# theovincent/iS-DQN

Hardware: AMD Instinct MI355X
Metric: gradient-steps/sec (batch=256, K=9, 84x84x4) (higher is better)
Workload: dtype bf16x3 (split-bf16 MFMA operands hi+lo, fp32 accumulate)

## Files before the change

is-dqn_amd/csrc/net_kernels.hip:

```cpp
#include <stdarg.h>
#include <stdlib.h>

#include <algorithm>
#include <type_traits>
#include <vector>
#include <atomic>

#include "conv_img.h"
#include "conv_u8_pair.h"
#include "conv_s8_pair.h"
#include "head_loss.h"
#include "munchausen.h"
#include "hl_gauss.h"
#include "quantile.h"
#include "categorical.h"
#include "net_plan.h"
#include "net_problems.h"

namespace isdqn {

__device__ inline double pow_int(double b, int t) {
    double r = 1.0, x = b;
    for (unsigned u = (unsigned)t; u != 0; u >>= 1) {
        if (u & 1u) r *= x;
// ... 315 lines not shown
    double* __restrict__ priorities = args.priorities;
    extern __shared__ float s_d[];
    __shared__ int s_action[TD_ROWS];
    const int tid = threadIdx.x, lane = tid & 63, wave = tid >> 6;
    const int b0 = blockIdx.x * TD_ROWS;
    const int b = b0 + lane;
    const bool on = b < B;
    float* s_td = s_d + TD_ROWS * K;
    const float inv_b = 1.f / (float)B;
    if (dout != nullptr) {
        const int rows = min(TD_ROWS, B - b0);
        for (int i = tid; i < rows * nha_p; i += 256) dout[(int64_t)b0 * nha_p + i] = 0.f;
    }
    int a = 0;
    float r = 0.f, nt = 0.f, w = 1.f;
    if (on) {
        a = action[b];
        r = reward[b];
        nt = 1.f - (float)terminal[b];
        if (loss_weights != nullptr) w = loss_weights[b];
    }
    if (wave == 0) s_action[lane] = on ? a : -1;
    for (int k = wave; k < K; k += 4) {
        float d = 0.f, td = 0.f;
        if (on) {
            float qv = q[(int64_t)b * nha_p + (oh + k) * A + a];
            const float* nq = vq + (int64_t)b * nha_p + (th + k) * A;
            float mx = nq[0];
            if (sq != nullptr) {
                const float* sel = sq + (int64_t)b * sq_pitch + (sh + k) * A;
                ISDQN_BOUNDS_CHECK(sel, 4 * A, 30);
                ISDQN_BOUNDS_CHECK(nq, 4 * A, 30);
                mx = nq[argmax_first(sel, A)];
            } else {
                for (int j = 1; j < A; ++j) mx = fmaxf(mx, nq[j]);
            }
            float tg = r + nt * gamma_n * mx;
            if (mq != nullptr) {
                const float* sv = mq + (int64_t)b * mq_pitch + (mh + k) * A;
                ISDQN_BOUNDS_CHECK(sv, 4 * A, 31);
                ISDQN_BOUNDS_CHECK(nq, 4 * A, 31);
                tg = munchausen_target(r, nt, gamma_n, sv[a], soft_value(sv, A, mu.tau), soft_value(nq, A, mu.tau), mu);
            }
            d = qv - tg;
            td = td_loss(d, huber_delta);
            if (q_values) q_values[(int64_t)b * K + k] = qv;
            if (targets) targets[(int64_t)b * K + k] = tg;
        }
        s_d[lane * K + k] = td_dloss(d, huber_delta) * inv_b * w;
        s_td[lane * K + k] = td;
        float sum = td * w;
        for (int off = 32; off > 0; off >>= 1) sum += __shfl_xor(sum, off);
        if (lane == 0) loss_part[(int64_t)blockIdx.x * K + k] = sum;
    }
    __syncthreads();
    if (dout != nullptr) {
        for (int i = tid; i < TD_ROWS * K; i += 256) {
            int bl = i / K, k = i - bl * K;
            if (b0 + bl < B) dout[(int64_t)(b0 + bl) * nha_p + (oh + k) * A + s_action[bl]] = s_d[i];
        }
        for (int c = tid; c < nha_p; c += 256) {
            float sum = 0.f;
            int head = c / A, aa = c - head * A;
            if (head >= oh && head < oh + K)
                for (int bl = 0; bl < TD_ROWS; ++bl) sum += (s_action[bl] == aa) ? s_d[bl * K + head - oh] : 0.f;
            dbh_part[(int64_t)blockIdx.x * nha_p + c] = sum;
        }
    }
    if (priorities != nullptr && tid < TD_ROWS && b0 + tid < B) {
        float sum = 0.f;
        for (int k = 0; k < K; ++k) sum += s_td[tid * K + k];
        priorities[b0 + tid] = sqrt((double)(sum / (float)K) + 1e-10);
    }
}

struct HeadChainParams {
    const float* slabs;
    int n_slabs;
    int64_t slab_stride, row_pitch;
    const float* hbias;
    float* act;
    float* z;
    const float* W;
    const float* bias;
    const float* gamma;
    const float* beta;
    int B, S, F, Fp, O, Op, K, A, oh;
    const int* action;
    const float* reward;
    const uint8_t* terminal;
    const float* loss_weights;
    float gamma_n, huber_delta;
    int double_q;
    Munchausen mu;
    float* dout;
    float* dz;
    float* part;
    float* q_values;
    float* targets;
    double* priorities;
    float* loss_part;
    float* dbh_part;
    int* adam_count;
    float b1, b2;
    float* adam_consts;
    long long* stamps;
};

constexpr int HC_MAX_COLS = 4;
constexpr int HC_THREADS = 512, HC_WAVES = HC_THREADS / 64;
constexpr int HC_KU = 16 / HC_WAVES;

__host__ __device__ inline int head_chain_pitch(int Fp) { return (Fp + 31) / 32 * 32 + 8; }
static inline int head_chain_lds_bytes(int Fp, int Op, int K, int passes, int S) {
    const int PA = head_chain_pitch(Fp);
    return (passes >= 2 ? 2 : 1) * 16 * PA * 2 + (HC_WAVES * 16 * Op + 16 * Op + S * Op + Op + 4 + 2 * S * Fp) * 4 + S * K * 12 +
           HC_WAVES * 2 * S * 2 * 4 + 64;
}

template <int PASSES, int COLS, int SMAX>
__global__ __launch_bounds__(HC_THREADS) void head_chain_kernel(const HeadChainParams p) {
    ISDQN_EMPTY_KERNEL_RETURN
    extern __shared__ __attribute__((aligned(16))) char hc_smem[];
    const int PA = head_chain_pitch(p.Fp);
    constexpr int A_PLANES = PASSES >= 2 ? 2 : 1;
    __bf16* a_hi = reinterpret_cast<__bf16*>(hc_smem);
    __bf16* a_lo = a_hi + 16 * PA;
    float* qpart = reinterpret_cast<float*>(a_hi + A_PLANES * 16 * PA);
    float* s_q = qpart + HC_WAVES * 16 * p.Op;
    float* s_dq = s_q + 16 * p.Op;
    float* s_d = s_dq + SMAX * p.Op;
    float* s_td = s_d + SMAX * p.K;
    float* s_wtd = s_td + SMAX * p.K;
    float* s_red = s_wtd + SMAX * p.K;
    float* s_bias = s_red + HC_WAVES * 2 * SMAX * 2;
    float* s_pre = reinterpret_cast<float*>((reinterpret_cast<uintptr_t>(s_bias + p.Op) + 15) & ~(uintptr_t)15);

    const int tid = threadIdx.x, lane = tid & 63, wave = tid >> 6;
#if defined(ISDQN_DEV)
#define HC_STAMP(i)                                                                                     \
    if (p.stamps != nullptr && threadIdx.x == 0) {                                                     \
        p.stamps[(int64_t)blockIdx.x * 8 + (i)] = (long long)__builtin_amdgcn_s_memtime();              \
        if ((i) == 0) p.stamps[(int64_t)blockIdx.x * 8 + 7] = (long long)__builtin_amdgcn_s_memrealtime(); \
    }
#else
#define HC_STAMP(i)
#endif
    HC_STAMP(0);
    const int S = p.S, b0 = (int)blockIdx.x * S;
    const int Fp = p.Fp, Op = p.Op, K = p.K, A = p.A;

    if (blockIdx.x == 0 && tid == 0) {
        int t = *p.adam_count + 1;
        *p.adam_count = t;
        p.adam_consts[0] = (float)(1.0 - pow_int((double)p.b1, t));
        p.adam_consts[1] = (float)(1.0 - pow_int((double)p.b2, t));
    }

    int act[SMAX];
#pragma unroll
    for (int s = 0; s < SMAX; ++s) {
        ISDQN_BOUNDS_CHECK((s < S && b0 + s < p.B) ? (const void*)(p.action + b0 + s) : zero_chunk(), 4, 20);
        act[s] = *(const ISDQN_GLOBAL int*)((s < S && b0 + s < p.B) ? (const void*)(p.action + b0 + s) : zero_chunk());
    }
    float td_r, td_w;
    uint8_t td_term;
    {
        const int s = tid / K;
        const bool ok = tid < S * K && b0 + s < p.B;
        const bool okw = ok && p.loss_weights != nullptr;
        ISDQN_BOUNDS_CHECK(okw ? (const void*)(p.loss_weights + b0 + s) : zero_chunk(), 4, 29);
        td_w = *(const ISDQN_GLOBAL float*)(okw ? (const void*)(p.loss_weights + b0 + s) : zero_chunk());
        ISDQN_BOUNDS_CHECK(ok ? (const void*)(p.reward + b0 + s) : zero_chunk(), 4, 21);
        ISDQN_BOUNDS_CHECK(ok ? (const void*)(p.terminal + b0 + s) : zero_chunk(), 1, 22);
        td_r = *(const ISDQN_GLOBAL float*)(ok ? (const void*)(p.reward + b0 + s) : zero_chunk());
        td_term = *(const ISDQN_GLOBAL uint8_t*)(ok ? (const void*)(p.terminal + b0 + s) : zero_chunk());
    }
    ISDQN_BOUNDS_CHECK(tid < p.O ? (const void*)(p.bias + tid) : zero_chunk(), 4, 23);
    const float bias_v = *(const ISDQN_GLOBAL float*)(tid < p.O ? (const void*)(p.bias + tid) : zero_chunk());
    float ga[COLS], be[COLS];
#pragma unroll
    for (int j = 0; j < COLS; ++j) {
        const int c = tid + j * HC_THREADS;
        const bool ok = p.gamma != nullptr && c < p.F;
        ISDQN_BOUNDS_CHECK(ok ? (const void*)(p.gamma + c) : zero_chunk(), 4, 24);
        ISDQN_BOUNDS_CHECK(ok ? (const void*)(p.beta + c) : zero_chunk(), 4, 24);
        ga[j] = *(const ISDQN_GLOBAL float*)(ok ? (const void*)(p.gamma + c) : zero_chunk());
        be[j] = *(const ISDQN_GLOBAL float*)(ok ? (const void*)(p.beta + c) : zero_chunk());
    }

    constexpr int R2 = 2 * SMAX;
    constexpr int TPR = HC_THREADS / R2;
    constexpr int SB = 32;
    static_assert(TPR % 64 == 0, "a wave must not straddle two rows");
    float m1 = 0.f, m2 = 0.f;
    {
        const int r = tid / TPR, q = tid - r * TPR;
        const int smp = r < S ? r : r - S;
        const bool row_ok = r < 2 * S && b0 + smp < p.B;
        const int64_t grow = r < S ? (int64_t)(b0 + smp) : (int64_t)p.B + b0 + smp;
        for (int c0 = q * 4; c0 < Fp; c0 += TPR * 4) {
            float hb4[4];
#pragma unroll
            for (int e = 0; e < 4; ++e) {
                ISDQN_BOUNDS_CHECK(c0 + e < p.F ? (const void*)(p.hbias + c0 + e) : zero_chunk(), 4, 25);
                hb4[e] = *(const ISDQN_GLOBAL float*)(c0 + e < p.F ? (const void*)(p.hbias + c0 + e) : zero_chunk());
            }
            const ISDQN_GLOBAL f32x4* base = (const ISDQN_GLOBAL f32x4*)(row_ok ? (const void*)(p.slabs + grow * p.row_pitch + c0) : zero_chunk());
            const int64_t strd = row_ok ? p.slab_stride / 4 : 0;
            f32x4 sum = f32x4{0.f, 0.f, 0.f, 0.f};
            for (int s0 = 0; s0 < p.n_slabs; s0 += SB) {
                f32x4 t[SB];
#pragma unroll
                for (int u = 0; u < SB; ++u) {
                    ISDQN_BOUNDS_CHECK((const void*)(base + min(s0 + u, p.n_slabs - 1) * strd), 16, 26);
                    t[u] = base[min(s0 + u, p.n_slabs - 1) * strd];
                }
#pragma unroll
                for (int u = 0; u < SB; ++u)
                    if (s0 + u < p.n_slabs) sum += t[u];
            }
            float v[4];
#pragma unroll
            for (int e = 0; e < 4; ++e) {
                v[e] = c0 + e < p.F ? sum[e] + hb4[e] : 0.f;
                m1 += v[e];
                m2 += v[e] * v[e];
            }
            *reinterpret_cast<float4*>(s_pre + r * Fp + c0) = make_float4(v[0], v[1], v[2], v[3]);
        }
    }

    HC_STAMP(6);
    const int nkt = (PA - 8) / 32, NT = (Op + 15) / 16;
    const int nks = (nkt + 15) / 16, n_items = ((NT + 1) / 2) * nks;
    const int kg8 = (lane >> 4) * 8;
    const int arow = (lane & 15) * PA + kg8;
    auto issue_w = [&](float (&v)[2][HC_KU][8], int item) {
        const int pair = item / nks, ksb = wave + 16 * (item - pair * nks);
#pragma unroll
        for (int t = 0; t < 2; ++t)
#pragma unroll
            for (int u = 0; u < HC_KU; ++u) {
                const int o = (pair * 2 + t) * 16 + (lane & 15), ks = ksb + HC_WAVES * u;
                const bool ok = item < n_items && o < p.O && ks < nkt && ks * 32 + kg8 < Fp;
                load8_aligned(ok ? p.W + (int64_t)o * Fp + ks * 32 + kg8 : zero_chunk(), v[t][u]);
            }
    };
    float wv0[2][HC_KU][8], wv1[2][HC_KU][8];
    issue_w(wv0, 0);

    float zv[SMAX][COLS];
    {
        for (int off = 32; off > 0; off >>= 1) {
            m1 += __shfl_xor(m1, off);
            m2 += __shfl_xor(m2, off);
        }
        if (lane == 0) {
            s_red[wave * 2] = m1;
            s_red[wave * 2 + 1] = m2;
        }
        __syncthreads();
        constexpr int WPR = TPR / 64;
#pragma unroll
        for (int r = 0; r < R2; ++r) {
            float a1 = s_red[r * WPR * 2], a2 = s_red[r * WPR * 2 + 1];
#pragma unroll
            for (int w = 1; w < WPR; ++w) {
                a1 += s_red[(r * WPR + w) * 2];
                a2 += s_red[(r * WPR + w) * 2 + 1];
            }
            const float mean = a1 / (float)p.F;
            const float rstd = rsqrtf(fmaxf(a2 / (float)p.F - mean * mean, 0.f) + 1e-6f);
            const int smp = r < S ? r : r - S;
            const bool row_ok = r < 2 * S && b0 + smp < p.B;
            const int64_t grow = r < S ? (int64_t)(b0 + smp) : (int64_t)p.B + b0 + smp;
#pragma unroll
            for (int j = 0; j < COLS; ++j) {
                const int c = tid + j * HC_THREADS;
                const float v = c < Fp ? s_pre[r * Fp + c] : 0.f;
                float y = v;
                if (p.gamma != nullptr && c < p.F) y = (v - mean) * (rstd * ga[j]) + be[j];
                y = fmaxf(y, 0.f);
                if (c >= p.F) y = 0.f;
                if (row_ok && c < Fp) {
                    s8_store_elem(p.act + grow * Fp, c, y);
                    if (r < S) p.z[grow * Fp + c] = v;
                }
                if (r < 2 * S && c < PA - 8) {
                    const float ys = row_ok ? y : 0.f;
                    const __bf16 h = (__bf16)ys;
                    a_hi[r * PA + c] = h;
                    if constexpr (PASSES >= 2) a_lo[r * PA + c] = (__bf16)(ys - (float)h);
                }
                if (r < SMAX) zv[r < SMAX ? r : 0][j] = (row_ok && r < S && c < p.F) ? v : 0.f;
            }
        }
    }
    for (int i = tid; i < SMAX * Op; i += HC_THREADS) s_dq[i] = 0.f;
    if (tid < Op) s_bias[tid] = bias_v;
    for (int o = tid + HC_THREADS; o < Op; o += HC_THREADS) s_bias[o] = o < p.O ? p.bias[o] : 0.f;
    __syncthreads();
    HC_STAMP(1);

    {
        f32x4 acc[2];
        auto run_item = [&](float (&v)[2][HC_KU][8], int item) {
            const int pair = item / nks, ksi = item - pair * nks, ksb = wave + 16 * ksi;
            if (ksi == 0) {
                acc[0] = acc[1] = f32x4{0.f, 0.f, 0.f, 0.f};
            }
#pragma unroll
            for (int u = 0; u < HC_KU; ++u) {
                const int ks = min(ksb + HC_WAVES * u, nkt - 1);
                const bf16x8 ah = *reinterpret_cast<const bf16x8*>(a_hi + arow + ks * 32);
                bf16x8 al;
                if constexpr (PASSES >= 2) al = *reinterpret_cast<const bf16x8*>(a_lo + arow + ks * 32);
#pragma unroll
                for (int t = 0; t < 2; ++t) {
                    bf16x8 bh, bl;
                    if constexpr (PASSES >= 2) {
                        split8(v[t][u], bh, bl);
                        if constexpr (PASSES >= 3)
                            mfma_acc(acc[t], ah, bl);
                        mfma_acc(acc[t], al, bh);
                    } else {
                        round8(v[t][u], bh);
                    }
                    mfma_acc(acc[t], ah, bh);
                }
            }
            const bool last = ksi + 1 == nks;
            if (last) {
#pragma unroll
                for (int t = 0; t < 2; ++t) {
                    const int o = (pair * 2 + t) * 16 + (lane & 15);
                    if (o < Op) {
#pragma unroll
                        for (int r = 0; r < 4; ++r) qpart[(wave * 16 + (lane >> 4) * 4 + r) * Op + o] = acc[t][r];
                    }
                }
            }
        };
        for (int item = 0; item < n_items; item += 2) {
            issue_w(wv1, item + 1);
            run_item(wv0, item);
            issue_w(wv0, item + 2);
            if (item + 1 < n_items) run_item(wv1, item + 1);
        }
    }

    auto issue_rows = [&](float (&w)[SMAX][4][COLS], int k0) {
#pragma unroll
        for (int s = 0; s < SMAX; ++s)
#pragma unroll
            for (int u = 0; u < 4; ++u) {
                const bool on = s < S && k0 + u < K;
                const float* wr = p.W + (int64_t)(on ? (p.oh + k0 + u) * A + act[s] : 0) * Fp;
#pragma unroll
                for (int j = 0; j < COLS; ++j) {
                    const int c = tid + j * HC_THREADS;
                    ISDQN_BOUNDS_CHECK(wr + (c < p.F ? c : 0), 4, 27);
                    w[s][u][j] = *(const ISDQN_GLOBAL float*)(wr + (c < p.F ? c : 0));
                }
            }
    };
    HC_STAMP(2);
    float wr0[SMAX][4][COLS], wr1[SMAX][4][COLS];
    issue_rows(wr0, 0);
    __syncthreads();
    for (int i = tid; i < 2 * S * Op; i += HC_THREADS) {
        const int o = i % Op;
        float v = qpart[i];
#pragma unroll
        for (int w = 1; w < HC_WAVES; ++w) v += qpart[w * 16 * Op + i];
        s_q[i] = o < p.O ? v + s_bias[o] : 0.f;
    }
    __syncthreads();

    const float inv_b = 1.f / (float)p.B;
    if (tid < S * K) {
        const int s = tid / K, k = tid - s * K;
        const int b = b0 + s;
        float d = 0.f, td = 0.f;
        int a = 0;
        if (b < p.B) {
            a = act[0];
#pragma unroll
            for (int i = 1; i < SMAX; ++i) a = s == i ? act[i] : a;
            const float qv = s_q[s * Op + (p.oh + k) * A + a];
            const float* nq = s_q + (S + s) * Op + k * A;
            float mx = nq[0];
            if (p.double_q) {
                mx = nq[argmax_first(nq + p.oh * A, A)];
            } else {
                for (int j = 1; j < A; ++j) mx = fmaxf(mx, nq[j]);
            }
            float tg = td_r + (1.f - (float)td_term) * p.gamma_n * mx;
            if (p.mu.tau > 0.f) {
                const float* sv = s_q + s * Op + k * A;
                tg = munchausen_target(td_r, 1.f - (float)td_term, p.gamma_n, sv[a], soft_value(sv, A, p.mu.tau), soft_value(nq, A, p.mu.tau), p.mu);
            }
            d = qv - tg;
            td = td_loss(d, p.huber_delta);
            if (p.q_values) p.q_values[(int64_t)b * K + k] = qv;
            if (p.targets) p.targets[(int64_t)b * K + k] = tg;
        }
        const float w = p.loss_weights != nullptr ? td_w : 1.f;
        const float dd = td_dloss(d, p.huber_delta) * inv_b * w;
        s_d[tid] = dd;
        s_td[tid] = td;
        s_wtd[tid] = td * w;
        s_dq[s * Op + (p.oh + k) * A + a] = dd;
    }
    __syncthreads();
    for (int i = tid; i < S * Op; i += HC_THREADS) {
        const int s = i / Op;
        if (b0 + s < p.B) p.dout[(int64_t)b0 * Op + i] = s_dq[i];
    }
    for (int c = tid; c < Op; c += HC_THREADS) {
        float sum = 0.f;
        for (int s = 0; s < S; ++s) sum += s_dq[s * Op + c];
        p.dbh_part[(int64_t)blockIdx.x * Op + c] = sum;
    }
    if (tid < K) {
        float sum = 0.f;
        for (int s = 0; s < S; ++s) sum += s_wtd[s * K + tid];
        p.loss_part[(int64_t)blockIdx.x * K + tid] = sum;
    }
    if (p.priorities != nullptr && tid < S && b0 + tid < p.B) {
        float sum = 0.f;
        for (int k = 0; k < K; ++k) sum += s_td[tid * K + k];
        p.priorities[b0 + tid] = sqrt((double)(sum / (float)K) + 1e-10);
    }

    HC_STAMP(3);
    float da[SMAX][COLS];
#pragma unroll
    for (int s = 0; s < SMAX; ++s)
#pragma unroll
        for (int j = 0; j < COLS; ++j) da[s][j] = 0.f;
    auto axpy_rows = [&](const float (&w)[SMAX][4][COLS], int k0) {
#pragma unroll
        for (int s = 0; s < SMAX; ++s)
#pragma unroll
            for (int u = 0; u < 4; ++u) {
                const bool on = s < S && k0 + u < K;
                const float dd = on ? s_d[s * K + k0 + u] : 0.f;
#pragma unroll
                for (int j = 0; j < COLS; ++j) da[s][j] += dd * w[s][u][j];
            }
    };
    for (int k0 = 0; k0 < K; k0 += 8) {
        issue_rows(wr1, k0 + 4);
        axpy_rows(wr0, k0);
        issue_rows(wr0, k0 + 8);
        if (k0 + 4 < K) axpy_rows(wr1, k0 + 4);
    }
    HC_STAMP(4);
    float dg[COLS], db[COLS], dbias[COLS];
#pragma unroll
    for (int j = 0; j < COLS; ++j) dg[j] = db[j] = dbias[j] = 0.f;
    if (p.gamma != nullptr) {
        const float inv_c = 1.f / (float)p.F;
        float r1[SMAX], r2[SMAX];
        auto block_sum2 = [&]() {
#pragma unroll
            for (int s = 0; s < SMAX; ++s)
                for (int off = 32; off > 0; off >>= 1) {
                    r1[s] += __shfl_xor(r1[s], off);
                    r2[s] += __shfl_xor(r2[s], off);
                }
            __syncthreads();
            if (lane == 0) {
#pragma unroll
                for (int s = 0; s < SMAX; ++s) {
                    s_red[(wave * SMAX + s) * 2] = r1[s];
                    s_red[(wave * SMAX + s) * 2 + 1] = r2[s];
                }
            }
            __syncthreads();
#pragma unroll
            for (int s = 0; s < SMAX; ++s) {
                r1[s] = s_red[s * 2];
                r2[s] = s_red[s * 2 + 1];
#pragma unroll
                for (int w = 1; w < HC_WAVES; ++w) {
                    r1[s] += s_red[(w * SMAX + s) * 2];
                    r2[s] += s_red[(w * SMAX + s) * 2 + 1];
                }
            }
        };
#pragma unroll
        for (int s = 0; s < SMAX; ++s) {
            r1[s] = r2[s] = 0.f;
#pragma unroll
            for (int j = 0; j < COLS; ++j) {
                r1[s] += zv[s][j];
                r2[s] += zv[s][j] * zv[s][j];
            }
        }
        block_sum2();
        float mean[SMAX], rstd[SMAX];
#pragma unroll
        for (int s = 0; s < SMAX; ++s) {
            mean[s] = r1[s] * inv_c;
            rstd[s] = rsqrtf(fmaxf(r2[s] * inv_c - mean[s] * mean[s], 0.f) + 1e-6f);
            r1[s] = r2[s] = 0.f;
#pragma unroll
            for (int j = 0; j < COLS; ++j) {
                const int c = tid + j * HC_THREADS;
                const bool ok = c < p.F && s < S && b0 + s < p.B;
                const float xh = (zv[s][j] - mean[s]) * rstd[s];
                const float y = xh * ga[j] + be[j];
                const float dy = (ok && y > 0.f) ? da[s][j] : 0.f;
                dg[j] += dy * xh;
                db[j] += dy;
                const float g2 = dy * ga[j];
                da[s][j] = g2;
                zv[s][j] = ok ? xh : 0.f;
                r1[s] += g2;
                r2[s] += g2 * zv[s][j];
            }
        }
        block_sum2();
#pragma unroll
        for (int s = 0; s < SMAX; ++s) {
            const float m1 = r1[s] * inv_c, m2 = r2[s] * inv_c;
            if (s < S && b0 + s < p.B) {
#pragma unroll
                for (int j = 0; j < COLS; ++j) {
                    const int c = tid + j * HC_THREADS;
                    if (c < Fp) {
                        const float o = c < p.F ? rstd[s] * (da[s][j] - m1 - zv[s][j] * m2) : 0.f;
                        dbias[j] += o;
                        s8_store_elem(p.dz + (int64_t)(b0 + s) * Fp, c, o);
                    }
                }
            }
        }
    } else {
#pragma unroll
        for (int s = 0; s < SMAX; ++s) {
            if (s < S && b0 + s < p.B) {
#pragma unroll
                for (int j = 0; j < COLS; ++j) {
                    const int c = tid + j * HC_THREADS;
                    if (c < Fp) {
                        const float o = (c < p.F && zv[s][j] > 0.f) ? da[s][j] : 0.f;
                        dbias[j] += o;
                        s8_store_elem(p.dz + (int64_t)(b0 + s) * Fp, c, o);
                    }
                }
            }
        }
    }
#pragma unroll
    for (int j = 0; j < COLS; ++j) {
        const int c = tid + j * HC_THREADS;
        if (c < Fp) {
            float* pp = p.part + (int64_t)blockIdx.x * 3 * Fp;
            pp[c] = dg[j];
            pp[Fp + c] = db[j];
            pp[2 * Fp + c] = dbias[j];
        }
    }
    HC_STAMP(5);
#undef HC_STAMP
}

__global__ __launch_bounds__(256) void loss_finalize_kernel(const float* __restrict__ loss_part,
                                                            const float* __restrict__ dbh_part, int n_blk, int B, int K,
                                                            int nha_p, float* __restrict__ losses,
                                                            float* __restrict__ loss_accum, float* __restrict__ dbh,
                                                            int* adam_count, float b1, float b2,
                                                            float* __restrict__ adam_consts) {
    ISDQN_EMPTY_KERNEL_RETURN
    const int tid = threadIdx.x, sub = tid & 15, grp = tid >> 4;
    const int nkb = (K + 15) / 16;
    const bool is_loss = (int)blockIdx.x < nkb;
    const int col = (is_loss ? (int)blockIdx.x : (int)blockIdx.x - nkb) * 16 + grp;
    const int ncol = is_loss ? K : nha_p;
    const float* src = is_loss ? loss_part : dbh_part;
    if (!is_loss && dbh == nullptr) return;
    float s = 0.f;
    if (col < ncol)
        for (int i0 = sub; i0 < n_blk; i0 += 8 * 16) {
            float v[8];
#pragma unroll
            for (int u = 0; u < 8; ++u) {
                const int i = i0 + u * 16;
                v[u] = i < n_blk ? src[(int64_t)i * ncol + col] : 0.f;
            }
#pragma unroll
            for (int u = 0; u < 8; ++u) s += v[u];
        }
    for (int off = 8; off > 0; off >>= 1) s += __shfl_xor(s, off);
    if (col < ncol && sub == 0) {
        if (is_loss) {
            s /= (float)B;
            losses[col] = s;
            if (loss_accum != nullptr) loss_accum[col] += s;
        } else {
            dbh[col] = s;
        }
    }
    if (blockIdx.x != 0) return;
    if (adam_count != nullptr && tid == 0) {
        int t = *adam_count + 1;
        *adam_count = t;
        adam_consts[0] = (float)(1.0 - pow_int((double)b1, t));
        adam_consts[1] = (float)(1.0 - pow_int((double)b2, t));
    }
}

struct AdamEntry {
    int64_t p_off, size, slab_stride;
    const float* g;
    int n_slabs, block_start;
};
constexpr int ADAM_MAX_ENTRIES = 4 * MAX_LAYERS;
struct AdamTable {
    AdamEntry e[ADAM_MAX_ENTRIES];
    int n, total_blocks;
};
__global__ __launch_bounds__(256) void adam_kernel(const AdamTable tab, float* __restrict__ p, float* __restrict__ m,
                                                   float* __restrict__ v, const float* __restrict__ consts, float lr,
                                                   float b1, float b2, float eps, float* __restrict__ grad_out,
                                                   float* __restrict__ mirror, int update) {
    ISDQN_EMPTY_KERNEL_RETURN
    __shared__ float4 s_g[16][16];
    int e = 0;
    while (e + 1 < tab.n && (int)blockIdx.x >= tab.e[e + 1].block_start) ++e;
    const AdamEntry en = tab.e[e];
    const float c1 = consts[0], c2 = consts[1];
    const int pos = threadIdx.x & 15, sl = threadIdx.x >> 4;
    const int64_t i = ((int64_t)(blockIdx.x - en.block_start) * 16 + pos) * 4;
    const bool on = i < en.size;
    float4 g = float4{0.f, 0.f, 0.f, 0.f};
    const int64_t o = en.p_off + i;
    float4 pm = g, pv = g, pp = g;
    if (on && sl == 0) {
        pm = *reinterpret_cast<const float4*>(m + o);
        pv = *reinterpret_cast<const float4*>(v + o);
        pp = *reinterpret_cast<const float4*>(p + o);
    }
    if (on) {
        int s = sl;
#if !defined(ISDQN_ADAM_4_IN_FLIGHT)
        for (; s + 7 * 16 < en.n_slabs; s += 8 * 16) {
// ... 955 lines not shown
};

static void head_chain_plan(LearnCtx& c, bool plan_heads) {
    const Plan& P = c.P;
    const Layer& hid = c.hid();
    static const bool hc_disabled = ISDQN_DEV_ENV("ISDQN_NO_HEAD_CHAIN");
    if (!(c.learn && c.update && plan_heads && !hc_disabled && c.target_params == nullptr && P.head_nb == 0 && P.n_layers >= 2 && hid.kind == 1 &&
          !hid.is_head && hid.has_relu && hid.out_p <= HC_THREADS * HC_MAX_COLS && hid.out_p % 8 == 0))
        return;
    const int S = c.B >= 1024 ? 4 : c.B >= 512 ? 2 : 1;
    const int n_wg = ceil_div(c.B, S);
    if (n_wg <= hid.part_rows && S * c.K <= HC_THREADS && head_chain_lds_bytes(hid.out_p, P.nha_p, c.K, c.x3 ? 3 : 1, S) <= 150 * 1024) {
        c.hc_S = S;
        c.hc_wg = n_wg;
    }
}

static int learn_forward(const LearnCtx& c) {
    const Plan& P = c.P;
    const isdqn_batch* batch = c.batch;
    float* ws = c.ws;
    const int B = c.B;
    int rc;
    if (c.target_params != nullptr && c.munchausen) {
        const int stack = c.cfg->arch != ISDQN_ARCH_FC ? c.cfg->obs_c : 0;
        rc = refresh_mirror(P, c.target_params, ws, c.st);
        if (rc) return rc;
        rc = net_forward(P, c.x3, c.target_params, c.in, P.N2, 0, ws, ws + P.out_t_off, c.st);
        if (rc) return rc;
        if (P.head_nb > 0) {
            rc = head_expect_rows(P, ws + P.logits_t_off, P.N2, ws + P.qt_off, c.st);
            if (rc) return rc;
        }
        rc = refresh_mirror(P, c.params, ws, c.st);
        if (rc) return rc;
        NetInput on{batch->frames, batch->frame_stride, batch->frame_ids, 0, batch->state, nullptr, 0, 2 * stack, 0};
        return net_forward(P, c.x3, c.params, on, B, B, ws, ws + P.out_off, c.st);
    }
    if (c.target_params != nullptr && c.double_q) {
        const int stack = c.cfg->arch != ISDQN_ARCH_FC ? c.cfg->obs_c : 0;
        NetInput nx{batch->frames, batch->frame_stride, batch->frame_ids, 0, batch->next_state, nullptr, 0, 2 * stack, stack};
        rc = refresh_mirror(P, c.target_params, ws, c.st);
        if (rc) return rc;
        rc = net_forward(P, c.x3, c.target_params, nx, B, 0, ws, ws + P.out_t_off, c.st);
        if (rc) return rc;
        if (P.head_nb > 0) {
            rc = head_expect_rows(P, ws + P.logits_t_off, B, ws + P.qt_off, c.st);
            if (rc) return rc;
        }
        rc = refresh_mirror(P, c.params, ws, c.st);
        if (rc) return rc;
        return net_forward(P, c.x3, c.params, c.in, P.N2, B, ws, ws + P.out_off, c.st);
    }
    if (c.target_params != nullptr) {
        const int stack = c.cfg->arch != ISDQN_ARCH_FC ? c.cfg->obs_c : 0;
        NetInput nx{batch->frames, batch->frame_stride, batch->frame_ids, 0, batch->next_state, nullptr, 0, 2 * stack, stack};
        rc = refresh_mirror(P, c.target_params, ws, c.st);
        if (rc) return rc;
        rc = net_forward(P, c.x3, c.target_params, nx, B, 0, ws, ws + P.out_off + (int64_t)B * P.nlog_p, c.st);
        if (rc) return rc;
        rc = refresh_mirror(P, c.params, ws, c.st);
        if (rc) return rc;
        NetInput on{batch->frames, batch->frame_stride, batch->frame_ids, 0, batch->state, nullptr, 0, 2 * stack, 0};
        return net_forward(P, c.x3, c.params, on, B, B, ws, ws + P.out_off, c.st);
    }
    if (!(batch->flags & ISDQN_BATCH_MIRROR_CURRENT)) {
        rc = refresh_mirror(P, c.params, ws, c.st);
        if (rc) return rc;
    }
    return net_forward(P, c.x3, c.params, c.in, P.N2, B, ws, ws + P.out_off, c.st, c.hc_S ? P.n_layers - 1 : -1, c.hc_S ? P.n_layers - 2 : -1);
}

static int launch_head_chain(const LearnCtx& c) {
    const Plan& P = c.P;
    const Layer &hid = c.hid(), &head = c.head();
    float* ws = c.ws;
    HeadChainParams hp;
    hp.act = ws + hid.act_off; hp.z = ws + hid.z_off;
    hp.slabs = ws + P.slab_off;
    hp.n_slabs = effective_splits(hid.in_unpadded_ld ? hid.in_f : hid.K, hid.fwd_splits);
    hp.slab_stride = hid.out_p;
    hp.row_pitch = (int64_t)hp.n_slabs * hid.out_p;
    hp.hbias = c.params + hid.b_off;
    hp.W = c.params + head.w_off; hp.bias = c.params + head.b_off;
    hp.gamma = hid.has_ln ? c.params + hid.g_off : nullptr;
    hp.beta = hid.has_ln ? c.params + hid.be_off : nullptr;
    hp.B = c.B; hp.S = c.hc_S; hp.F = hid.out_f; hp.Fp = hid.out_p; hp.O = P.nha; hp.Op = P.nha_p; hp.K = c.K; hp.oh = P.oh;
    hp.A = P.n_actions;
    hp.action = c.batch->action; hp.reward = c.batch->reward; hp.terminal = c.batch->terminal;
    hp.loss_weights = c.batch->loss_weights;
    hp.gamma_n = c.cfg->gamma_n; hp.huber_delta = c.cfg->huber_delta;
    hp.double_q = c.double_q ? 1 : 0;
    hp.mu = Munchausen{c.cfg->munchausen_tau, c.cfg->munchausen_alpha, c.cfg->munchausen_clip};
    hp.dout = ws + P.dout_off; hp.dz = ws + hid.dz_off; hp.part = ws + hid.part_off;
    hp.q_values = c.qv; hp.targets = c.tg; hp.priorities = c.priorities;
    hp.loss_part = ws + P.lpart_off; hp.dbh_part = hp.loss_part + (int64_t)c.hc_wg * c.K;
    hp.adam_count = c.adam_count; hp.b1 = c.cfg->adam_b1; hp.b2 = c.cfg->adam_b2; hp.adam_consts = ws + P.adam_tab_off;
    hp.stamps = stamps_for("head_chain");
    const int lds = head_chain_lds_bytes(hid.out_p, P.nha_p, c.K, c.x3 ? 3 : 1, c.hc_S);
    const int cols = ceil_div(hid.out_p, HC_THREADS) <= 1 ? 1 : ceil_div(hid.out_p, HC_THREADS) <= 2 ? 2 : 4;
    auto launch_hc = [&](auto kern, int slot) -> int {
        static LdsConfigured configured[18];
        if (int rc2 = ensure_dynamic_lds(kern, lds, configured[slot])) return rc2;
        ISDQN_REPORT_OCCUPANCY(kern, HC_THREADS, lds, c.hc_wg);
        hipLaunchKernelGGL(kern, dim3(c.hc_wg), dim3(HC_THREADS), lds, c.st, hp);
        ISDQN_HIP_CHECK(hipGetLastError());
        return ISDQN_OK;
    };
    auto by_cols = [&](auto passes_c, auto s_c, int base) -> int {
        constexpr int PS = decltype(passes_c)::value, SS = decltype(s_c)::value;
        return cols == 1 ? launch_hc(&head_chain_kernel<PS, 1, SS>, base) : cols == 2 ? launch_hc(&head_chain_kernel<PS, 2, SS>, base + 1)
                                                                        : launch_hc(&head_chain_kernel<PS, 4, SS>, base + 2);
    };
    auto by_s = [&](auto passes_c, int base) -> int {
        return c.hc_S == 1 ? by_cols(passes_c, std::integral_constant<int, 1>{}, base)
             : c.hc_S == 2 ? by_cols(passes_c, std::integral_constant<int, 2>{}, base + 3)
                           : by_cols(passes_c, std::integral_constant<int, 4>{}, base + 6);
    };
    return c.x3 ? by_s(std::integral_constant<int, 3>{}, 0) : by_s(std::integral_constant<int, 1>{}, 9);
}

static int head_chain_sums(const LearnCtx& c, hipStream_t s) {
    return loss_finalize(c.P, c.cfg, c.ws, c.hc_wg, c.K, c.P.nha_p, c.losses, c.loss_accum, true, nullptr, s);
}
static int head_chain_tail(const LearnCtx& c, hipStream_t s) {
    if (int rc = head_chain_sums(c, s)) return rc;
    const Layer& head = c.head();
    return dense_wgrad(head, c.x3, c.in, c.ws + c.hid().act_off, c.ws + c.P.dout_off, c.P.nlog_p, c.ws + head.gw_off, c.B, s);
}

static int learn_loss(const LearnCtx& c) {
    const bool tnet = (c.double_q || c.munchausen) && c.target_params != nullptr;
    if (!c.hc_S)
        return loss_and_finalize(c.P, c.cfg, c.ws, c.batch, c.K, c.on0, c.tg0, c.learn, (c.learn && c.update) ? c.adam_count : nullptr, c.qv, c.tg,
                                 c.priorities, c.losses, c.loss_accum, c.st, c.double_q,
                                 tnet ? c.ws + c.P.out_t_off + (c.munchausen ? (int64_t)c.B * c.P.nlog_p : 0) : nullptr,
                                 (tnet && c.munchausen) ? c.ws + c.P.out_t_off : nullptr);
    if (int rc = launch_head_chain(c)) return rc;
    return c.ss ? ISDQN_OK : head_chain_sums(c, c.st);
}

struct WgradJob {
    int layer = -1;
    hipStream_t stream = nullptr;
    hipEvent_t wait = nullptr;
    const float* dz = nullptr;
    int dz_ld = 0;
};

static int dense_wgrad_fused_adam(const LearnCtx& c, const Layer& l, const float* act_in, const WgradJob& j) {
    const MatSrc A{j.dz, j.dz_ld, c.B, l.out_p, 1};
    const MatSrc Bm{act_in, l.in_p, c.B, l.in_p, 1};
    AdamFuse af{c.params + l.w_off, c.adam_m + l.w_off, c.adam_v + l.w_off, c.ws + c.P.adam_tab_off,
                c.cfg->learning_rate, c.cfg->adam_b1, c.cfg->adam_b2, c.cfg->adam_eps,
                c.grad_out ? c.grad_out + l.w_off : nullptr, c.ws + c.P.wsplit_off + l.w_off, c.update ? 1 : 0};
    if (l.is_head)
        return c.x3 ? launch_plain<64, 64, 2, 2, true, true, 3, true, false, true, 2>(A, nullptr, 0, Bm, nullptr, l.in_p, l.out_p, l.in_p, c.B, 1, 0,
                                                                                      j.stream, &af)
                    : launch_plain<64, 64, 2, 2, true, true, 1, true, false, true, 2>(A, nullptr, 0, Bm, nullptr, l.in_p, l.out_p, l.in_p, c.B, 1, 0,
                                                                                      j.stream, &af);
    return c.x3 ? launch_plain<64, 64, 2, 2, true, true, 3, true, false, true, DZ_S8 | 2>(A, nullptr, 0, Bm, nullptr, l.in_p, l.out_p, l.in_p, c.B, 1,
                                                                                          0, j.stream, &af)
                : launch_plain<64, 64, 2, 2, true, true, 1, true, false, true, DZ_S8 | 2>(A, nullptr, 0, Bm, nullptr, l.in_p, l.out_p, l.in_p, c.B, 1,
                                                                                          0, j.stream, &af);
}

static int weight_gradient(const LearnCtx& c, const WgradJob& j, AdamList* adam) {
// ... 534 lines not shown
```

Measured before the change: 4283.

## Overlap head-chain weight prefetch with slab reduction and parallelize target max

Moves the head-weight loads to a pre-split bf16 mirror (Wmir) and issues them, together with a three-deep ring of weight tiles and, for single-sample blocks, the action rows, during the tail of the slab-reduction loop. It also adds a shuffle-based parallel max/argmax over actions for the TD target that skips the separate s_q reduction pass and one barrier. Smaller changes: the Adam step counter update moves later in the kernel, the slab batch size and the number of rows fetched per step shrink, and timing stamps are buffered in registers and written once at the end. The intent is to hide global-memory latency and remove the split/round work and a synchronisation step, at the cost of more register pressure and reliance on the mirror staying in sync with the weights.

Result: no change. 4297, median of 2 (+0.3%).

```diff
diff --git a/is-dqn_amd/csrc/net_kernels.hip b/is-dqn_amd/csrc/net_kernels.hip
--- a/is-dqn_amd/csrc/net_kernels.hip
+++ b/is-dqn_amd/csrc/net_kernels.hip
@@ -421,6 +421,7 @@
     float* act;
     float* z;
     const float* W;
+    const float* Wmir;
     const float* bias;
     const float* gamma;
     const float* beta;
@@ -473,14 +474,15 @@
     float* s_wtd = s_td + SMAX * p.K;
     float* s_red = s_wtd + SMAX * p.K;
     float* s_bias = s_red + HC_WAVES * 2 * SMAX * 2;
-    float* s_pre = reinterpret_cast<float*>((reinterpret_cast<uintptr_t>(s_bias + p.Op) + 15) & ~(uintptr_t)15);
+    float* s_pre = reinterpret_cast<float*>(hc_smem + (((reinterpret_cast<char*>(s_bias + p.Op) - hc_smem) + 15) & ~(ptrdiff_t)15));
 
     const int tid = threadIdx.x, lane = tid & 63, wave = tid >> 6;
 #if defined(ISDQN_DEV)
-#define HC_STAMP(i)                                                                                     \
-    if (p.stamps != nullptr && threadIdx.x == 0) {                                                     \
-        p.stamps[(int64_t)blockIdx.x * 8 + (i)] = (long long)__builtin_amdgcn_s_memtime();              \
-        if ((i) == 0) p.stamps[(int64_t)blockIdx.x * 8 + 7] = (long long)__builtin_amdgcn_s_memrealtime(); \
+    long long hc_t[8] = {0, 0, 0, 0, 0, 0, 0, 0};
+#define HC_STAMP(i)                                                              \
+    if (p.stamps != nullptr && threadIdx.x == 0) {                               \
+        hc_t[(i)] = (long long)__builtin_amdgcn_s_memtime();                     \
+        if ((i) == 0) hc_t[7] = (long long)__builtin_amdgcn_s_memrealtime();     \
     }
 #else
 #define HC_STAMP(i)
@@ -489,24 +491,21 @@
     const int S = p.S, b0 = (int)blockIdx.x * S;
     const int Fp = p.Fp, Op = p.Op, K = p.K, A = p.A;
 
-    if (blockIdx.x == 0 && tid == 0) {
-        int t = *p.adam_count + 1;
-        *p.adam_count = t;
-        p.adam_consts[0] = (float)(1.0 - pow_int((double)p.b1, t));
-        p.adam_consts[1] = (float)(1.0 - pow_int((double)p.b2, t));
-    }
-
     int act[SMAX];
 #pragma unroll
     for (int s = 0; s < SMAX; ++s) {
         ISDQN_BOUNDS_CHECK((s < S && b0 + s < p.B) ? (const void*)(p.action + b0 + s) : zero_chunk(), 4, 20);
         act[s] = *(const ISDQN_GLOBAL int*)((s < S && b0 + s < p.B) ? (const void*)(p.action + b0 + s) : zero_chunk());
     }
+    int tgt_g = 1, tgt_sh = 0;
+    while (tgt_g < A) { tgt_g <<= 1; ++tgt_sh; }
+    const bool tgt_par = !(p.mu.tau > 0.f) && A <= 64 && S * K * tgt_g <= HC_THREADS;
+    const int pair_id = tgt_par ? tid >> tgt_sh : tid, pair_lane = tgt_par ? tid & (tgt_g - 1) : 0;
     float td_r, td_w;
     uint8_t td_term;
     {
-        const int s = tid / K;
-        const bool ok = tid < S * K && b0 + s < p.B;
+        const int s = pair_id / K;
+        const bool ok = pair_id < S * K && b0 + s < p.B;
         const bool okw = ok && p.loss_weights != nullptr;
         ISDQN_BOUNDS_CHECK(okw ? (const void*)(p.loss_weights + b0 + s) : zero_chunk(), 4, 29);
         td_w = *(const ISDQN_GLOBAL float*)(okw ? (const void*)(p.loss_weights + b0 + s) : zero_chunk());
@@ -530,35 +529,91 @@
 
     constexpr int R2 = 2 * SMAX;
     constexpr int TPR = HC_THREADS / R2;
-    constexpr int SB = 32;
+    constexpr int SB = 16;
     static_assert(TPR % 64 == 0, "a wave must not straddle two rows");
+    const int nkt = (PA - 8) / 32, NT = (Op + 15) / 16;
+    const int nks = (nkt + 15) / 16, n_items = ((NT + 1) / 2) * nks;
+    const int kg8 = (lane >> 4) * 8;
+    const int arow = (lane & 15) * PA + kg8;
+    constexpr int WN = PASSES >= 2 ? 8 : 4;
+    auto issue_w = [&](float (&v)[2][HC_KU][WN], int item) {
+        const int pair = item / nks, ksb = wave + 16 * (item - pair * nks);
+#pragma unroll
+        for (int t = 0; t < 2; ++t)
+#pragma unroll
+            for (int u = 0; u < HC_KU; ++u) {
+                const int o = (pair * 2 + t) * 16 + (lane & 15), ks = ksb + HC_WAVES * u;
+                const bool ok = item < n_items && o < p.O && ks < nkt && ks * 32 + kg8 < Fp;
+                const float* src = ok ? p.Wmir + (int64_t)o * Fp + ks * 32 + kg8 : zero_chunk();
+                ISDQN_BOUNDS_CHECK(src, 4 * WN, 36);
+#pragma unroll
+                for (int h = 0; h < WN / 4; ++h) {
+                    const f32x4 x = ((const ISDQN_GLOBAL f32x4*)src)[h];
+                    v[t][u][h * 4] = x[0]; v[t][u][h * 4 + 1] = x[1]; v[t][u][h * 4 + 2] = x[2]; v[t][u][h * 4 + 3] = x[3];
+                }
+            }
+    };
+    constexpr int HC_RING = 3;
+    float wv0[2][HC_KU][WN], wv1[2][HC_KU][WN], wv2[2][HC_KU][WN];
+    constexpr int HC_ROWS_AHEAD = SMAX == 1 ? 16 / COLS : 0;
+    const bool rows_ahead = SMAX == 1 && K <= HC_ROWS_AHEAD;
+    float wra[HC_ROWS_AHEAD > 0 ? HC_ROWS_AHEAD : 1][COLS];
+    auto issue_ahead = [&]() {
+        issue_w(wv0, 0);
+        issue_w(wv1, 1);
+        issue_w(wv2, 2);
+        if constexpr (HC_ROWS_AHEAD > 0) {
+#pragma unroll
+            for (int k = 0; k < HC_ROWS_AHEAD; ++k) {
+                const bool on = rows_ahead && k < K;
+                const float* wr = p.W + (int64_t)(on ? (p.oh + k) * A + act[0] : 0) * Fp;
+#pragma unroll
+                for (int j = 0; j < COLS; ++j) {
+                    const int c = tid + j * HC_THREADS;
+                    ISDQN_BOUNDS_CHECK(wr + (c < p.F ? c : 0), 4, 27);
+                    wra[k][j] = *(const ISDQN_GLOBAL float*)(wr + (c < p.F ? c : 0));
+                }
+            }
+        }
+    };
     float m1 = 0.f, m2 = 0.f;
     {
         const int r = tid / TPR, q = tid - r * TPR;
         const int smp = r < S ? r : r - S;
         const bool row_ok = r < 2 * S && b0 + smp < p.B;
         const int64_t grow = r < S ? (int64_t)(b0 + smp) : (int64_t)p.B + b0 + smp;
-        for (int c0 = q * 4; c0 < Fp; c0 += TPR * 4) {
+        auto slab_pass = [&](int c0, auto&& behind) {
+            const bool col_ok = c0 < Fp;
             float hb4[4];
 #pragma unroll
             for (int e = 0; e < 4; ++e) {
                 ISDQN_BOUNDS_CHECK(c0 + e < p.F ? (const void*)(p.hbias + c0 + e) : zero_chunk(), 4, 25);
                 hb4[e] = *(const ISDQN_GLOBAL float*)(c0 + e < p.F ? (const void*)(p.hbias + c0 + e) : zero_chunk());
             }
-            const ISDQN_GLOBAL f32x4* base = (const ISDQN_GLOBAL f32x4*)(row_ok ? (const void*)(p.slabs + grow * p.row_pitch + c0) : zero_chunk());
-            const int64_t strd = row_ok ? p.slab_stride / 4 : 0;
+            const ISDQN_GLOBAL f32x4* base = (const ISDQN_GLOBAL f32x4*)(row_ok && col_ok ? (const void*)(p.slabs + grow * p.row_pitch + c0) : zero_chunk());
+            const int64_t strd = row_ok && col_ok ? p.slab_stride / 4 : 0;
             f32x4 sum = f32x4{0.f, 0.f, 0.f, 0.f};
-            for (int s0 = 0; s0 < p.n_slabs; s0 += SB) {
-                f32x4 t[SB];
+            f32x4 t[SB];
+            auto request = [&](int s0) {
 #pragma unroll
                 for (int u = 0; u < SB; ++u) {
                     ISDQN_BOUNDS_CHECK((const void*)(base + min(s0 + u, p.n_slabs - 1) * strd), 16, 26);
                     t[u] = base[min(s0 + u, p.n_slabs - 1) * strd];
                 }
+            };
+            auto add = [&](int s0) {
 #pragma unroll
                 for (int u = 0; u < SB; ++u)
                     if (s0 + u < p.n_slabs) sum += t[u];
-            }
+            };
+            int s0 = 0;
+            for (; s0 + SB < p.n_slabs; s0 += SB) {
+                request(s0);
+                add(s0);
+            }
+            request(s0);
+            behind();
+            add(s0);
             float v[4];
 #pragma unroll
             for (int e = 0; e < 4; ++e) {
@@ -566,28 +621,15 @@
                 m1 += v[e];
                 m2 += v[e] * v[e];
             }
-            *reinterpret_cast<float4*>(s_pre + r * Fp + c0) = make_float4(v[0], v[1], v[2], v[3]);
-        }
+            if (col_ok) *reinterpret_cast<float4*>(s_pre + r * Fp + c0) = make_float4(v[0], v[1], v[2], v[3]);
+        };
+        int c0 = q * 4;
+        for (; c0 + TPR * 4 < Fp; c0 += TPR * 4) slab_pass(c0, [] {});
+        if (__builtin_amdgcn_ballot_w64(c0 < Fp) != 0) slab_pass(c0, issue_ahead);
+        else issue_ahead();
     }
 
     HC_STAMP(6);
-    const int nkt = (PA - 8) / 32, NT = (Op + 15) / 16;
-    const int nks = (nkt + 15) / 16, n_items = ((NT + 1) / 2) * nks;
-    const int kg8 = (lane >> 4) * 8;
-    const int arow = (lane & 15) * PA + kg8;
-    auto issue_w = [&](float (&v)[2][HC_KU][8], int item) {
-        const int pair = item / nks, ksb = wave + 16 * (item - pair * nks);
-#pragma unroll
-        for (int t = 0; t < 2; ++t)
-#pragma unroll
-            for (int u = 0; u < HC_KU; ++u) {
-                const int o = (pair * 2 + t) * 16 + (lane & 15), ks = ksb + HC_WAVES * u;
-                const bool ok = item < n_items && o < p.O && ks < nkt && ks * 32 + kg8 < Fp;
-                load8_aligned(ok ? p.W + (int64_t)o * Fp + ks * 32 + kg8 : zero_chunk(), v[t][u]);
-            }
-    };
-    float wv0[2][HC_KU][8], wv1[2][HC_KU][8];
-    issue_w(wv0, 0);
 
     float zv[SMAX][COLS];
     {
@@ -641,10 +683,16 @@
     for (int o = tid + HC_THREADS; o < Op; o += HC_THREADS) s_bias[o] = o < p.O ? p.bias[o] : 0.f;
     __syncthreads();
     HC_STAMP(1);
+    if (blockIdx.x == 0 && tid == 0) {
+        int t = *p.adam_count + 1;
+        *p.adam_count = t;
+        p.adam_consts[0] = (float)(1.0 - pow_int((double)p.b1, t));
+        p.adam_consts[1] = (float)(1.0 - pow_int((double)p.b2, t));
+    }
 
     {
         f32x4 acc[2];
-        auto run_item = [&](float (&v)[2][HC_KU][8], int item) {
+        auto run_item = [&](float (&v)[2][HC_KU][WN], int item) {
             const int pair = item / nks, ksi = item - pair * nks, ksb = wave + 16 * ksi;
             if (ksi == 0) {
                 acc[0] = acc[1] = f32x4{0.f, 0.f, 0.f, 0.f};
@@ -659,12 +707,12 @@
                 for (int t = 0; t < 2; ++t) {
                     bf16x8 bh, bl;
                     if constexpr (PASSES >= 2) {
-                        split8(v[t][u], bh, bl);
+                        s8_unpack(v[t][u], bh, bl);
                         if constexpr (PASSES >= 3)
                             mfma_acc(acc[t], ah, bl);
                         mfma_acc(acc[t], al, bh);
                     } else {
-                        round8(v[t][u], bh);
+                        bh = __builtin_bit_cast(bf16x8, f32x4{v[t][u][0], v[t][u][1], v[t][u][2], v[t][u][3]});
                     }
                     mfma_acc(acc[t], ah, bh);
                 }
@@ -676,24 +724,31 @@
                     const int o = (pair * 2 + t) * 16 + (lane & 15);
                     if (o < Op) {
 #pragma unroll
-                        for (int r = 0; r < 4; ++r) qpart[(wave * 16 + (lane >> 4) * 4 + r) * Op + o] = acc[t][r];
+                        for (int r = 0; r < 4; ++r) {
+                            const int row = (lane >> 4) * 4 + r;
+                            if (row < 2 * S) qpart[(wave * 16 + row) * Op + o] = acc[t][r];
+                        }
                     }
                 }
             }
         };
-        for (int item = 0; item < n_items; item += 2) {
-            issue_w(wv1, item + 1);
+        for (int item = 0; item < n_items; item += HC_RING) {
+            const bool more = item + HC_RING < n_items;
             run_item(wv0, item);
-            issue_w(wv0, item + 2);
+            if (more) issue_w(wv0, item + 3);
             if (item + 1 < n_items) run_item(wv1, item + 1);
-        }
-    }
-
-    auto issue_rows = [&](float (&w)[SMAX][4][COLS], int k0) {
+            if (more) issue_w(wv1, item + 4);
+            if (item + 2 < n_items) run_item(wv2, item + 2);
+            if (more) issue_w(wv2, item + 5);
+        }
+    }
+
+    constexpr int HB = SMAX * COLS >= 16 ? 2 : 4;
+    auto issue_rows = [&](float (&w)[SMAX][HB][COLS], int k0) {
 #pragma unroll
         for (int s = 0; s < SMAX; ++s)
 #pragma unroll
-            for (int u = 0; u < 4; ++u) {
+            for (int u = 0; u < HB; ++u) {
                 const bool on = s < S && k0 + u < K;
                 const float* wr = p.W + (int64_t)(on ? (p.oh + k0 + u) * A + act[s] : 0) * Fp;
 #pragma unroll
@@ -705,52 +760,89 @@
             }
     };
     HC_STAMP(2);
-    float wr0[SMAX][4][COLS], wr1[SMAX][4][COLS];
-    issue_rows(wr0, 0);
+    float wr0[SMAX][HB][COLS], wr1[SMAX][HB][COLS];
+    if (!rows_ahead) issue_rows(wr0, 0);
     __syncthreads();
-    for (int i = tid; i < 2 * S * Op; i += HC_THREADS) {
-        const int o = i % Op;
-        float v = qpart[i];
-#pragma unroll
-        for (int w = 1; w < HC_WAVES; ++w) v += qpart[w * 16 * Op + i];
-        s_q[i] = o < p.O ? v + s_bias[o] : 0.f;
-    }
-    __syncthreads();
 
     const float inv_b = 1.f / (float)p.B;
-    if (tid < S * K) {
-        const int s = tid / K, k = tid - s * K;
-        const int b = b0 + s;
+    auto td_tail = [&](int pr, int s, int k, int a, bool live, float qv, float tg) {
         float d = 0.f, td = 0.f;
-        int a = 0;
-        if (b < p.B) {
-            a = act[0];
-#pragma unroll
-            for (int i = 1; i < SMAX; ++i) a = s == i ? act[i] : a;
-            const float qv = s_q[s * Op + (p.oh + k) * A + a];
-            const float* nq = s_q + (S + s) * Op + k * A;
-            float mx = nq[0];
-            if (p.double_q) {
-                mx = nq[argmax_first(nq + p.oh * A, A)];
-            } else {
-                for (int j = 1; j < A; ++j) mx = fmaxf(mx, nq[j]);
-            }
-            float tg = td_r + (1.f - (float)td_term) * p.gamma_n * mx;
-            if (p.mu.tau > 0.f) {
-                const float* sv = s_q + s * Op + k * A;
-                tg = munchausen_target(td_r, 1.f - (float)td_term, p.gamma_n, sv[a], soft_value(sv, A, p.mu.tau), soft_value(nq, A, p.mu.tau), p.mu);
-            }
+        if (live) {
             d = qv - tg;
             td = td_loss(d, p.huber_delta);
-            if (p.q_values) p.q_values[(int64_t)b * K + k] = qv;
-            if (p.targets) p.targets[(int64_t)b * K + k] = tg;
+            if (p.q_values) p.q_values[(int64_t)(b0 + s) * K + k] = qv;
+            if (p.targets) p.targets[(int64_t)(b0 + s) * K + k] = tg;
         }
         const float w = p.loss_weights != nullptr ? td_w : 1.f;
         const float dd = td_dloss(d, p.huber_delta) * inv_b * w;
-        s_d[tid] = dd;
-        s_td[tid] = td;
-        s_wtd[tid] = td * w;
+        s_d[pr] = dd;
+        s_td[pr] = td;
+        s_wtd[pr] = td * w;
         s_dq[s * Op + (p.oh + k) * A + a] = dd;
+    };
+    if (tgt_par) {
+        auto q_at = [&](int row, int o) {
+            float v = qpart[row * Op + o];
+#pragma unroll
+            for (int w = 1; w < HC_WAVES; ++w) v += qpart[(w * 16 + row) * Op + o];
+            return o < p.O ? v + s_bias[o] : 0.f;
+        };
+        const int pr = min(pair_id, S * K - 1), s = pr / K, k = pr - s * K;
+        const int j = min(pair_lane, A - 1);
+        int a = act[0];
+#pragma unroll
+        for (int i = 1; i < SMAX; ++i) a = s == i ? act[i] : a;
+        const bool live = b0 + s < p.B;
+        if (!live) a = 0;
+        const float qv = q_at(s, (p.oh + k) * A + a);
+        float mx = q_at(S + s, k * A + j);
+        if (p.double_q) {
+            float sv = q_at(S + s, (p.oh + k) * A + j);
+            int si = j;
+            for (int off = tgt_g >> 1; off > 0; off >>= 1) {
+                const float ov = __shfl_xor(sv, off);
+                const int oi = __shfl_xor(si, off);
+                if (ov > sv || (ov == sv && oi < si)) { sv = ov; si = oi; }
+            }
+            mx = __shfl(mx, (lane & ~(tgt_g - 1)) + si);
+        } else {
+            for (int off = tgt_g >> 1; off > 0; off >>= 1) mx = fmaxf(mx, __shfl_xor(mx, off));
+        }
+        if (pair_lane == 0 && pair_id < S * K) td_tail(pr, s, k, a, live, qv, td_r + (1.f - (float)td_term) * p.gamma_n * mx);
+    } else {
+        for (int i = tid; i < 2 * S * Op; i += HC_THREADS) {
+            const int o = i % Op;
+            float v = qpart[i];
+#pragma unroll
+            for (int w = 1; w < HC_WAVES; ++w) v += qpart[w * 16 * Op + i];
+            s_q[i] = o < p.O ? v + s_bias[o] : 0.f;
+        }
+        __syncthreads();
+        if (tid < S * K) {
+            const int s = tid / K, k = tid - s * K;
+            const bool live = b0 + s < p.B;
+            float qv = 0.f, tg = 0.f;
+            int a = 0;
+            if (live) {
+                a = act[0];
+#pragma unroll
+                for (int i = 1; i < SMAX; ++i) a = s == i ? act[i] : a;
+                qv = s_q[s * Op + (p.oh + k) * A + a];
+                const float* nq = s_q + (S + s) * Op + k * A;
+                float mx = nq[0];
+                if (p.double_q) {
+                    mx = nq[argmax_first(nq + p.oh * A, A)];
+                } else {
+                    for (int j = 1; j < A; ++j) mx = fmaxf(mx, nq[j]);
+                }
+                tg = td_r + (1.f - (float)td_term) * p.gamma_n * mx;
+                if (p.mu.tau > 0.f) {
+                    const float* sv = s_q + s * Op + k * A;
+                    tg = munchausen_target(td_r, 1.f - (float)td_term, p.gamma_n, sv[a], soft_value(sv, A, p.mu.tau), soft_value(nq, A, p.mu.tau), p.mu);
+                }
+            }
+            td_tail(tid, s, k, a, live, qv, tg);
+        }
     }
     __syncthreads();
     for (int i = tid; i < S * Op; i += HC_THREADS) {
@@ -779,22 +871,33 @@
     for (int s = 0; s < SMAX; ++s)
 #pragma unroll
         for (int j = 0; j < COLS; ++j) da[s][j] = 0.f;
-    auto axpy_rows = [&](const float (&w)[SMAX][4][COLS], int k0) {
+    auto axpy_rows = [&](const float (&w)[SMAX][HB][COLS], int k0) {
 #pragma unroll
         for (int s = 0; s < SMAX; ++s)
 #pragma unroll
-            for (int u = 0; u < 4; ++u) {
+            for (int u = 0; u < HB; ++u) {
                 const bool on = s < S && k0 + u < K;
                 const float dd = on ? s_d[s * K + k0 + u] : 0.f;
 #pragma unroll
                 for (int j = 0; j < COLS; ++j) da[s][j] += dd * w[s][u][j];
             }
     };
-    for (int k0 = 0; k0 < K; k0 += 8) {
-        issue_rows(wr1, k0 + 4);
-        axpy_rows(wr0, k0);
-        issue_rows(wr0, k0 + 8);
-        if (k0 + 4 < K) axpy_rows(wr1, k0 + 4);
+    if (rows_ahead) {
+        if constexpr (HC_ROWS_AHEAD > 0) {
+#pragma unroll
+            for (int k = 0; k < HC_ROWS_AHEAD; ++k) {
+                const float dd = k < K ? s_d[k] : 0.f;
+#pragma unroll
+                for (int j = 0; j < COLS; ++j) da[0][j] += dd * wra[k][j];
+            }
+        }
+    } else {
+        for (int k0 = 0; k0 < K; k0 += 2 * HB) {
+            issue_rows(wr1, k0 + HB);
+            axpy_rows(wr0, k0);
+            issue_rows(wr0, k0 + 2 * HB);
+            if (k0 + HB < K) axpy_rows(wr1, k0 + HB);
+        }
     }
     HC_STAMP(4);
     float dg[COLS], db[COLS], dbias[COLS];
@@ -905,6 +1008,12 @@
         }
     }
     HC_STAMP(5);
+#if defined(ISDQN_DEV)
+    if (p.stamps != nullptr && threadIdx.x == 0) {
+#pragma unroll
+        for (int i = 0; i < 8; ++i) p.stamps[(int64_t)blockIdx.x * 8 + i] = hc_t[i];
+    }
+#endif
 #undef HC_STAMP
 }
 
@@ -2027,6 +2136,7 @@
     hp.row_pitch = (int64_t)hp.n_slabs * hid.out_p;
     hp.hbias = c.params + hid.b_off;
     hp.W = c.params + head.w_off; hp.bias = c.params + head.b_off;
+    hp.Wmir = c.wmir() + head.w_off;
     hp.gamma = hid.has_ln ? c.params + hid.g_off : nullptr;
     hp.beta = hid.has_ln ? c.params + hid.be_off : nullptr;
     hp.B = c.B; hp.S = c.hc_S; hp.F = hid.out_f; hp.Fp = hid.out_p; hp.O = P.nha; hp.Op = P.nha_p; hp.K = c.K; hp.oh = P.oh;
```

## Read head weights from pre-split mirror and exact-size slab reduction loop

Applied to the files above, without the earlier changes.

The head-chain kernel now loads the head weight matrix from a pre-split mirror buffer (Wm) and unpacks its hi/lo bf16 halves with s8_unpack. This replaces the per-use split8/round8 conversion from fp32. The slab reduction over split-K partials drops the fixed 32-wide clamped batches. It uses 16-wide, then 4-wide, then single-slab chunks, so clamped duplicate loads and predicated adds go away. The change depends on the mirror being kept current and matching the packed layout that s8_unpack expects.

New measurement: 4247 before, 4280 after, median of 6. No clear change (+0.8%).

```diff
diff --git a/is-dqn_amd/csrc/net_kernels.hip b/is-dqn_amd/csrc/net_kernels.hip
--- a/is-dqn_amd/csrc/net_kernels.hip
+++ b/is-dqn_amd/csrc/net_kernels.hip
@@ -421,6 +421,7 @@
     float* act;
     float* z;
     const float* W;
+    const float* Wm;
     const float* bias;
     const float* gamma;
     const float* beta;
@@ -530,7 +531,7 @@
 
     constexpr int R2 = 2 * SMAX;
     constexpr int TPR = HC_THREADS / R2;
-    constexpr int SB = 32;
+    constexpr int SB = 16, SB_TAIL = 4;
     static_assert(TPR % 64 == 0, "a wave must not straddle two rows");
     float m1 = 0.f, m2 = 0.f;
     {
@@ -548,17 +549,21 @@
             const ISDQN_GLOBAL f32x4* base = (const ISDQN_GLOBAL f32x4*)(row_ok ? (const void*)(p.slabs + grow * p.row_pitch + c0) : zero_chunk());
             const int64_t strd = row_ok ? p.slab_stride / 4 : 0;
             f32x4 sum = f32x4{0.f, 0.f, 0.f, 0.f};
-            for (int s0 = 0; s0 < p.n_slabs; s0 += SB) {
-                f32x4 t[SB];
-#pragma unroll
-                for (int u = 0; u < SB; ++u) {
-                    ISDQN_BOUNDS_CHECK((const void*)(base + min(s0 + u, p.n_slabs - 1) * strd), 16, 26);
-                    t[u] = base[min(s0 + u, p.n_slabs - 1) * strd];
+            auto add_slabs = [&](auto n_c, int s0) {
+                constexpr int N = decltype(n_c)::value;
+                f32x4 t[N];
+#pragma unroll
+                for (int u = 0; u < N; ++u) {
+                    ISDQN_BOUNDS_CHECK((const void*)(base + (s0 + u) * strd), 16, 26);
+                    t[u] = base[(s0 + u) * strd];
                 }
 #pragma unroll
-                for (int u = 0; u < SB; ++u)
-                    if (s0 + u < p.n_slabs) sum += t[u];
-            }
+                for (int u = 0; u < N; ++u) sum += t[u];
+            };
+            int s0 = 0;
+            for (; s0 + SB <= p.n_slabs; s0 += SB) add_slabs(std::integral_constant<int, SB>{}, s0);
+            for (; s0 + SB_TAIL <= p.n_slabs; s0 += SB_TAIL) add_slabs(std::integral_constant<int, SB_TAIL>{}, s0);
+            for (; s0 < p.n_slabs; ++s0) add_slabs(std::integral_constant<int, 1>{}, s0);
             float v[4];
 #pragma unroll
             for (int e = 0; e < 4; ++e) {
@@ -583,7 +588,9 @@
             for (int u = 0; u < HC_KU; ++u) {
                 const int o = (pair * 2 + t) * 16 + (lane & 15), ks = ksb + HC_WAVES * u;
                 const bool ok = item < n_items && o < p.O && ks < nkt && ks * 32 + kg8 < Fp;
-                load8_aligned(ok ? p.W + (int64_t)o * Fp + ks * 32 + kg8 : zero_chunk(), v[t][u]);
+                const float* src = ok ? p.Wm + (int64_t)o * Fp + ks * 32 + kg8 : zero_chunk();
+                ISDQN_BOUNDS_CHECK(src, 32, 36);
+                load8_aligned(src, v[t][u]);
             }
     };
     float wv0[2][HC_KU][8], wv1[2][HC_KU][8];
@@ -659,12 +666,12 @@
                 for (int t = 0; t < 2; ++t) {
                     bf16x8 bh, bl;
                     if constexpr (PASSES >= 2) {
-                        split8(v[t][u], bh, bl);
+                        s8_unpack(v[t][u], bh, bl);
                         if constexpr (PASSES >= 3)
                             mfma_acc(acc[t], ah, bl);
                         mfma_acc(acc[t], al, bh);
                     } else {
-                        round8(v[t][u], bh);
+                        s8_unpack_hi(v[t][u], bh);
                     }
                     mfma_acc(acc[t], ah, bh);
                 }
@@ -2026,7 +2033,7 @@
     hp.slab_stride = hid.out_p;
     hp.row_pitch = (int64_t)hp.n_slabs * hid.out_p;
     hp.hbias = c.params + hid.b_off;
-    hp.W = c.params + head.w_off; hp.bias = c.params + head.b_off;
+    hp.W = c.params + head.w_off; hp.Wm = c.wmir() + head.w_off; hp.bias = c.params + head.b_off;
     hp.gamma = hid.has_ln ? c.params + hid.g_off : nullptr;
     hp.beta = hid.has_ln ? c.params + hid.be_off : nullptr;
     hp.B = c.B; hp.S = c.hc_S; hp.F = hid.out_f; hp.Fp = hid.out_p; hp.O = P.nha; hp.Op = P.nha_p; hp.K = c.K; hp.oh = P.oh;
```
